# Hitenze/Preconditioned_Additive_Gaussian_Processes_with_Fourier_Acceleration

Measured on AMD Instinct MI355X. Metric: kernel matvecs/sec + PCG wall-time to 1e-6, n=1e6 d=32 additive, 1/2/4/8 GPU, higher is better.
Workload: dtype f64; 1 GPU; additive NFFT matvec, n=1000000, d=32, 32 x 1-D windows, Gaussian f=1 l=1 mu=0.01 (BASELINE configs[2]); n=1000000, d=32, nwindows=32, parallelism=single

## Files before the change

### preconditioned_additive_gaussian_processes_with_fourier_acceleration_amd/csrc/nfft_kernels.hip

```cpp
#include <hip/hip_ext.h>
#include <hip/hip_runtime.h>

#include <algorithm>
#include <cmath>
#include <cstdio>
#include <vector>

#include "internal.h"
#include "reduce.hpp"

namespace nfft4gp_amd {

constexpr int kGridThreads = 1024;
constexpr int kMomStride = kNC + 1;
constexpr int kMomWin = kNC * kNos + 4;
template <int MOMT>
__host__ __device__ constexpr int mom_doubles_per_window()
{
   return MOMT ? kMomWin : kNos * kMomStride;
}
template <int MOMT>
__device__ __forceinline__ int mom_index(int cl, int cell, int d)
{
   return MOMT ? cl * kMomWin + d * kNos + cell : (cl * kNos + cell) * kMomStride + d;
// ... 617 lines not shown
   for (size_t j0 = (size_t)blockIdx.x * kGridThreads + tid; j0 < (size_t)n; j0 += kU * stride) {
      double xv[kU], yv[kU];
#pragma unroll
      for (int u = 0; u < kU; u++) {
         const size_t j = j0 + u * stride;
         xv[u] = j < (size_t)n ? x[j] : 0.0;
         yv[u] = (beta != 0.0 && j < (size_t)n) ? y[j] : 0.0;
      }
#pragma unroll
      for (int u = 0; u < kU; u++) {
         const size_t j = j0 + u * stride;
         if (j < (size_t)n) y[j] = (beta == 0.0 ? 0.0 : beta * yv[u]) + amu * xv[u];
      }
   }
   if (A.bufs) peer_gather(A, comp, s_g);
   __syncthreads();
   grid_tail(comp, s_g, wv, ct, H, s_w, s_h);
}

template <int THREADS, int REC = 5>
__global__ __launch_bounds__(THREADS) void k_interp_part(const uint16_t* __restrict__ meta,
                                                        const uint32_t* __restrict__ lo,
                                                        const uint32_t* __restrict__ qarr,
                                                        const int* __restrict__ tile_off, const double* __restrict__ H,
                                                        double* __restrict__ y, int n, int B, int ngroups, int S,
                                                        double scale)
{
   extern __shared__ __attribute__((aligned(16))) double smem[];
   double* s_y = smem;
   const int b = blockIdx.x / S, part = blockIdx.x % S;
   const int g0 = part * ngroups / S, g1 = (part + 1) * ngroups / S;
   const int tid = threadIdx.x;
   const int base = b * B;
   const int nloc = min(B, n - base);
   TileRegs cur;
   const int t1 = tile_off[b * ngroups + g1];
   int t = tile_at<REC>(cur, meta, lo, qarr, tile_off[b * ngroups + g0] + (tid >> 6), t1);
   for (int i = tid; i < B + kPad; i += THREADS) s_y[i] = 0.0;
   __syncthreads();
   for (; t < t1; t = tile_at<REC>(cur, meta, lo, qarr, t + THREADS / 64, t1)) {
      double h[kNC];
      gather_h(h, H, cur.mt);
      interp_run<REC, false>(cur, h, 0.0);
   }
   __syncthreads();
   for (int j = tid; j < nloc; j += THREADS) atomicAdd(y + (size_t)base + j, scale * s_y[j]);
}

__global__ __launch_bounds__(kGridThreads) void k_reduce_parts(const double* __restrict__ part, int nparts, int nw,
                                                              double* __restrict__ gsum, PeerArgs A)
{
   __shared__ double s_red[kGridThreads];
   const int comp = blockIdx.x;
   const int tid = threadIdx.x;
   const double v = parts_sum(part, nparts, comp, s_red);
   if (tid < kNos) {
      if (A.bufs)
         peer_put(A, comp, tid, v);
      else
         gsum[(size_t)comp * kNos + tid] = v;
   }
}

template <bool GRAD, int THREADS, bool DOT = false, bool DET = false, int REC = 5>
__global__ __launch_bounds__(THREADS) void k_interp(
    const uint16_t* __restrict__ meta, const uint32_t* __restrict__ lo, const uint32_t* __restrict__ qarr,
    const int* __restrict__ tile_off, const double* __restrict__ H, const double* __restrict__ Hd,
    const double* __restrict__ x, double* __restrict__ y, int n, int B, int ngroups, double alpha, double beta,
    double f, double mu, double dg, double* __restrict__ dot_part, unsigned int* __restrict__ dot_ticket,
    double* __restrict__ dot_out, const double* __restrict__ hb, int nw)
{
   extern __shared__ __attribute__((aligned(16))) double smem[];
   const int Bp = B + kPad;
   double* s_y = smem;
   double* s_yd = smem + Bp;
   const int b = blockIdx.x;
   const int tid = threadIdx.x;
   const int base = b * B;
   const int nloc = min(B, n - base);
   if constexpr (GRAD) {
      const int lane = tid & 63;
      const int wave = tid >> 6;
      constexpr int nwaves = THREADS / 64;
      const int t0 = tile_off[b * ngroups];
      const int t1 = tile_off[(b + 1) * ngroups];
      TileRegs cur;
      int t = tile_at<REC>(cur, meta, lo, qarr, t0 + wave, t1);
      const bool ep_regs = B <= kEpMax * THREADS;
      double xe[kEpMax];
      if (ep_regs) {
#pragma unroll
         for (int k = 0; k < kEpMax; k++) {
            const int j = tid + k * THREADS;
            xe[k] = (j < nloc) ? x[(size_t)base + j] : 0.0;
         }
      }
      for (int i = tid; i < Bp; i += THREADS) {
         s_y[i] = 0.0;
         s_yd[i] = 0.0;
      }
      const double Cy = DET ? det_grid(det_interp_exp(hb, nw)) : 0.0;
      const double Cyd = DET ? det_grid(det_interp_exp(hb + nw, nw)) : 0.0;
      __syncthreads();

      for (; t < t1; t += nwaves) {
         const int tn = t + nwaves;
         const size_t hoff = (size_t)cur.mt * kNC;
         double hc[kNC], hdc[kNC];
#pragma unroll
         for (int d = 0; d < kNC; d += 2) {
            const double2 v = *reinterpret_cast<const double2*>(H + hoff + d);
            hc[d] = v.x;
            hc[d + 1] = v.y;
            const double2 vd = *reinterpret_cast<const double2*>(Hd + hoff + d);
            hdc[d] = vd.x;
            hdc[d + 1] = vd.y;
         }
#pragma unroll
         for (int r = 0; r < kR; r++) {
            const uint32_t off = slot_off<REC>(cur, r);
            const double u = q_to_s(cur.qq[r]);
            double v = hc[kNC - 1];
#pragma unroll
            for (int d = kNC - 2; d >= 0; d--) v = fma(v, u, hc[d]);
            lds_add(off, DET ? det_round(v, Cy) : v);
            double vd = hdc[kNC - 1];
#pragma unroll
            for (int d = kNC - 2; d >= 0; d--) vd = fma(vd, u, hdc[d]);
            lds_add(off + 8u * (uint32_t)Bp, DET ? det_round(vd, Cyd) : vd);
         }
         if (tn < t1) load_tile<REC>(cur, meta, lo, qarr, tn, lane);
      }
      __syncthreads();

      const double ff = f * f;
      double* y0 = y;
      double* y1 = y + n;
      double* y2 = y + 2 * (size_t)n;
#pragma unroll
      for (int k = 0; k < kEpMax; k++) {
         if (!ep_regs) break;
         const int j = tid + k * THREADS;
         if (j >= nloc) break;
         const size_t gj = (size_t)base + j;
         const double xj = xe[k];
         const double v0 = 2.0 * f * (s_y[j] + mu * xj);
         const double v1 = ff * s_yd[j];
         const double v2 = dg * ff * xj;
         if (beta == 0.0) {
            y0[gj] = alpha * v0;
            y1[gj] = alpha * v1;
            y2[gj] = alpha * v2;
         } else {
            y0[gj] = fma(beta, y0[gj], alpha * v0);
            y1[gj] = fma(beta, y1[gj], alpha * v1);
            y2[gj] = fma(beta, y2[gj], alpha * v2);
         }
      }
      if (!ep_regs) {
         for (int j = tid; j < nloc; j += THREADS) {
            const size_t gj = (size_t)base + j;
            const double xj = x[gj];
            const double v0 = 2.0 * f * (s_y[j] + mu * xj);
            const double v1 = ff * s_yd[j];
            const double v2 = dg * ff * xj;
            if (beta == 0.0) {
               y0[gj] = alpha * v0;
               y1[gj] = alpha * v1;
               y2[gj] = alpha * v2;
            } else {
               y0[gj] = fma(beta, y0[gj], alpha * v0);
               y1[gj] = fma(beta, y1[gj], alpha * v1);
               y2[gj] = fma(beta, y2[gj], alpha * v2);
            }
         }
      }
      return;
   }
   TileRegs cur;
   const int t1 = tile_off[(b + 1) * ngroups];
   int t = tile_at<REC>(cur, meta, lo, qarr, tile_off[b * ngroups] + (tid >> 6), t1);
   double xe[kEpMax], ye[kEpMax];
   ep_prefetch<THREADS>(xe, ye, x, y, base, nloc, beta);
   for (int i = tid; i < Bp; i += THREADS) s_y[i] = 0.0;
   const double Cy = DET ? det_grid(det_interp_exp(hb, nw)) : 0.0;
   __syncthreads();

   for (; t < t1; t = tile_at<REC>(cur, meta, lo, qarr, t + THREADS / 64, t1)) {
      double h[kNC];
      gather_h(h, H, cur.mt);
      interp_run<REC, DET>(cur, h, Cy);
   }
   __syncthreads();

   const double dacc = ep_plain<THREADS, DOT>(xe, ye, s_y, y, base, nloc, alpha, beta, f, mu);
   if (DOT) ep_dot_finish<THREADS>(dacc, smem + Bp, dot_part, dot_ticket, dot_out);
}

constexpr int kHlWin = kNC * kNos + 1;
constexpr size_t kMaxDynamicLds = 160 * 1024;

__host__ __device__ constexpr size_t hl_lds_bytes(int B, int CG, int ngroups, int ns)
{
   return sizeof(double) * ((size_t)B + kPad) + sizeof(double) * (size_t)ns * CG * kHlWin +
          sizeof(int) * (1 + (size_t)ns + 2 * (size_t)ngroups);
}

__device__ __forceinline__ void hl_stage_wave(double* s_H, const double* __restrict__ H, int g, int slot, int CG, int nw,
                                              int lane)
{
   const int c0 = g * CG;
   const int ncomp = min(CG, nw - c0);
   const double2* src = reinterpret_cast<const double2*>(H + (size_t)c0 * kNos * kNC);
   double* dst = s_H + (size_t)slot * CG * kHlWin;
   const int pairs = ncomp * kNos * kNC / 2;
#pragma unroll 4
   for (int i = lane; i < pairs; i += 64) {
      const double2 v = src[i];
      const int e = 2 * i;
      const int cl = e / (kNos * kNC);
      const int cell = (e / kNC) & (kNos - 1);
      const int d = e & (kNC - 1);
      double* row = dst + cl * kHlWin + cell;
      row[d * kNos] = v.x;
      row[(d + 1) * kNos] = v.y;
   }
}

template <int THREADS, bool DET = false, int REC = 5>
__global__ __launch_bounds__(THREADS) void k_interp_hl(const uint16_t* __restrict__ meta, const uint32_t* __restrict__ lo,
                                                       const uint32_t* __restrict__ qarr, const int* __restrict__ tile_off,
                                                       const double* __restrict__ H, const double* __restrict__ x,
                                                       double* __restrict__ y, int n, int B, int ngroups, int CG, int nw,
                                                       double alpha, double beta, double f, double mu,
                                                       const double* __restrict__ hb, int ns)
{
   extern __shared__ __attribute__((aligned(16))) double smem[];
   const int Bp = B + kPad;
   double* s_y = smem;
   double* s_H = smem + Bp;
   int* s_ready = reinterpret_cast<int*>(s_H + (size_t)ns * CG * kHlWin);
   int* s_done = s_ready + ns;
   int* s_toff = s_done + ngroups;
   const int b = blockIdx.x;
   const int tid = threadIdx.x;
   const int base = b * B;
   const int nloc = min(B, n - base);
   const int lane = tid & 63;
   const int wave = tid >> 6;
   constexpr int nwaves = THREADS / 64;
   const int gbase = b * ngroups;
   TileRegs cur;
   const int t1 = tile_off[gbase + ngroups];
   int t = tile_at<REC>(cur, meta, lo, qarr, tile_off[gbase] + wave, t1);
   double xe[kEpMax], ye[kEpMax];
   ep_prefetch<THREADS>(xe, ye, x, y, base, nloc, beta);
   for (int i = tid; i < Bp; i += THREADS) s_y[i] = 0.0;
   for (int i = tid; i < ngroups; i += THREADS) s_done[i] = 0;
   for (int i = tid; i <= ngroups; i += THREADS) s_toff[i] = tile_off[gbase + i];
   if (tid < ns) s_ready[tid] = tid;
   if (wave < ns && wave < ngroups) hl_stage_wave(s_H, H, wave, wave, CG, nw, lane);
   const double Cy = DET ? det_grid(det_interp_exp(hb, nw)) : 0.0;
   __syncthreads();

   int g = 0, gslot = 0;
   int gend = s_toff[1];
   auto leave = [&](int gl) {
      int old = 0;
      if (lane == 0) old = __hip_atomic_fetch_add(s_done + gl, 1, __ATOMIC_ACQ_REL, __HIP_MEMORY_SCOPE_WORKGROUP);
      old = __builtin_amdgcn_readfirstlane(old);
      if (old == nwaves - 1 && gl + ns < ngroups) {
         const int sl = gl % ns;
         hl_stage_wave(s_H, H, gl + ns, sl, CG, nw, lane);
         __builtin_amdgcn_fence(__ATOMIC_RELEASE, "workgroup");
         if (lane == 0) __hip_atomic_store(s_ready + sl, gl + ns, __ATOMIC_RELEASE, __HIP_MEMORY_SCOPE_WORKGROUP);
      }
   };
   for (; t < t1; t = tile_at<REC>(cur, meta, lo, qarr, t + nwaves, t1)) {
      while (t >= gend) {
         leave(g);
         g++;
         gend = s_toff[g + 1];
         gslot = g % ns;
         if (g >= ns) {
            for (long spin = 0; spin < (1l << 24); spin++) {
               if (__hip_atomic_load(s_ready + gslot, __ATOMIC_ACQUIRE, __HIP_MEMORY_SCOPE_WORKGROUP) == g) break;
               __builtin_amdgcn_s_sleep(1);
            }
         }
      }
      const int cl = (int)(cur.mt >> 6) - g * CG;
      const int cell = (int)(cur.mt & 63u);
      double h[kNC];
      gather_h_lds(h, s_H + ((size_t)gslot * CG + cl) * kHlWin + cell, kNos);
      interp_run<REC, DET>(cur, h, Cy);
   }
   for (; g < ngroups; g++) leave(g);
   __syncthreads();

   ep_plain<THREADS, false>(xe, ye, s_y, y, base, nloc, alpha, beta, f, mu);
}

constexpr int kFgWin = kNC * kFgCells + 1;
constexpr int kFgRow = kNos + 1;
constexpr int kFgQuads = (kFgSpan + 3) / 4;
constexpr int kFgHs = 4 * kFgQuads + 1;
constexpr int kFgLdsWin = kFgWin + kFgHs + 2 * kFgRow;

template <int THREADS, bool DOT = false, int REC = 5, bool TIMELINE = false>
__global__ __launch_bounds__(THREADS) void k_interp_fg(
    const uint16_t* __restrict__ meta, const uint32_t* __restrict__ lo, const uint32_t* __restrict__ qarr,
    const int* __restrict__ tile_off, const double* __restrict__ gsum, double* __restrict__ gclear,
    const double* __restrict__ wcirc, const double* __restrict__ x, double* __restrict__ y, int n, int B, int ngroups,
    double alpha, double beta, double f, double mu, double* __restrict__ dot_part,
    unsigned int* __restrict__ dot_ticket, double* __restrict__ dot_out, int nw)
{
   static_assert(THREADS % (4 * kNC) == 0 && kNC == 8, "a thread keeps its degree and cell quarter over the build");
   static_assert(kFgSpan % 6 == 0, "the circulant's steps go six per trip");
   extern __shared__ __attribute__((aligned(16))) double smem[];
   const int Bp = B + kPad;
   double* s_y = smem;
   double* s_H = smem + Bp;
   double* s_h = s_H + (size_t)nw * kFgWin;
   double* s_g = s_h + (size_t)nw * kFgHs;
   double* s_w = s_g + (size_t)nw * kFgRow;
   double* s_scr = s_w + (size_t)nw * kFgRow;
   const int b = blockIdx.x;
   const int tid = threadIdx.x;
   const int base = b * B;
   const int nloc = min(B, n - base);
   constexpr int nwaves = THREADS / 64;
   if (TIMELINE) stamp(0);
   const int t1 = tile_off[(b + 1) * ngroups];
   int t = tile_off[b * ngroups] + (tid >> 6);
   constexpr int kFgRegTrips = 2;
   const int ns = nw * kNos;
   double gv[kFgRegTrips], wv[kFgRegTrips];
#pragma unroll
   for (int k = 0; k < kFgRegTrips; k++) {
      const int i = min(tid + k * THREADS, ns - 1);
      gv[k] = gsum[i];
      wv[k] = wcirc[i];
   }
   double ct[kTaps];
#pragma unroll
   for (int tp = 0; tp < kTaps; tp++) ct[tp] = c_taps[tp * kNC + (tid & (kNC - 1))];
   for (int i = tid + kFgRegTrips * THREADS; i < ns; i += THREADS) {
      const int o = (i >> 6) * kFgRow + (i & (kNos - 1));
      s_g[o] = gsum[i];
      s_w[o] = wcirc[i];
   }
   TileRegs cur, nxt;
   __builtin_amdgcn_sched_barrier(0);
   load_tile<REC>(cur, meta, lo, qarr, max(min(t, t1 - 1), 0), tid & 63);
   __builtin_amdgcn_sched_barrier(0);
   for (int i = tid; i < Bp; i += THREADS) s_y[i] = 0.0;
#pragma unroll
   for (int k = 0; k < kFgRegTrips; k++) {
      const int i = tid + k * THREADS;
      if (i < ns) {
         const int o = (i >> 6) * kFgRow + (i & (kNos - 1));
         s_g[o] = gv[k];
         s_w[o] = wv[k];
      }
   }
   if (b == 0)
      for (int i = tid; i < ns; i += THREADS) gclear[i] = 0.0;
   __syncthreads();
   if (TIMELINE) stamp(1);
   for (int it = tid; it < nw * kFgQuads; it += THREADS) {
      const int w = it / kFgQuads, k0 = 4 * (it % kFgQuads);
      const double* gw = s_g + w * kFgRow;
      const double* ww = s_w + w * kFgRow;
      double r3 = ww[(k0 + 3) & (kNos - 1)], r2 = ww[(k0 + 2) & (kNos - 1)], r1 = ww[(k0 + 1) & (kNos - 1)], r0 = ww[k0];
      double a0 = 0.0, a1 = 0.0, a2 = 0.0, a3 = 0.0;
#pragma unroll 6
      for (int j = 0; j < kFgSpan; j++) {
         const double gj = gw[(kFgSpan0 + j) & (kNos - 1)];
         a0 = fma(r0, gj, a0);
         a1 = fma(r1, gj, a1);
         a2 = fma(r2, gj, a2);
         a3 = fma(r3, gj, a3);
         r3 = r2, r2 = r1, r1 = r0;
         r0 = ww[(k0 - j - 1) & (kNos - 1)];
      }
      double* hw = s_h + w * kFgHs + k0;
      hw[0] = a0, hw[1] = a1, hw[2] = a2, hw[3] = a3;
   }
   load_tile<REC>(nxt, meta, lo, qarr, max(min(t + nwaves, t1 - 1), 0), tid & 63);
   __syncthreads();
   {
      const int d = tid & (kNC - 1), seg = (tid >> 3) & 3;
      const int c0 = seg ? 8 * seg + 1 : 0, c1 = 8 * seg + 9;
      for (int w = tid >> 5; w < nw; w += THREADS / 32) {
         const double* hw = s_h + w * kFgHs + c0;
         double hv[kTaps + 8];
#pragma unroll
         for (int j = 0; j < kTaps + 8; j++) hv[j] = hw[j];
         double acc[9];
#pragma unroll
         for (int k = 0; k < 9; k++) acc[k] = 0.0;
#pragma unroll
         for (int tp = 0; tp < kTaps; tp++) {
#pragma unroll
            for (int k = 0; k < 9; k++) acc[k] = fma(hv[k + tp], ct[tp], acc[k]);
         }
         double* dst = s_H + (size_t)w * kFgWin + d * kFgCells + c0;
#pragma unroll
         for (int k = 0; k < 9; k++)
            if (c0 + k < c1) dst[k] = acc[k];
      }
   }
   __syncthreads();
   if (TIMELINE) stamp(2);
   double xe[kEpMax], ye[kEpMax];
   ep_prefetch<THREADS>(xe, ye, x, y, base, nloc, beta);

   auto run = [&](const TileRegs& T) {
      const int ci = min((int)((T.mt + 16u) & 63u), kFgCells - 1);
      double h[kNC];
      gather_h_lds(h, s_H + (size_t)(T.mt >> 6) * kFgWin + ci, kFgCells);
      interp_run<REC, false>(T, h, 0.0);
   };
   if (t < t1) {
      run(cur);
      const int tn = t + nwaves;
      t = t1;
      if (tn < t1) {
         t = tile_at<REC>(cur, meta, lo, qarr, tn + nwaves, t1);
         run(nxt);
      }
   }
   for (; t < t1; t = tile_at<REC>(cur, meta, lo, qarr, t + nwaves, t1)) run(cur);
   __syncthreads();
   if (TIMELINE) stamp(3);

   const double dacc = ep_plain<THREADS, DOT, true>(xe, ye, s_y, y, base, nloc, alpha, beta, f, mu);
   if (DOT) ep_dot_finish<THREADS>(dacc, s_scr, dot_part, dot_ticket, dot_out);
}


template <int THREADS, bool DET = false, int REC = 5>
__global__ __launch_bounds__(THREADS) void k_interp2(const uint16_t* __restrict__ meta,
                                                     const uint32_t* __restrict__ lo,
                                                     const uint32_t* __restrict__ qarr,
                                                     const int* __restrict__ tile_off, const double* __restrict__ H,
                                                     size_t h_rs, const double* __restrict__ x0,
                                                     const double* __restrict__ x1, double* __restrict__ y0,
                                                     double* __restrict__ y1, int n, int B, int ngroups, double alpha,
                                                     double beta, double f, double mu, const double* __restrict__ hb,
                                                     int nw)
{
   extern __shared__ __attribute__((aligned(16))) double smem[];
   const int Bp = B + kPad;
   double* s_y0 = smem;
   double* s_y1 = smem + Bp;
   const int b = blockIdx.x;
   const int tid = threadIdx.x;
   const int base = b * B;
   const int nloc = min(B, n - base);
   const int lane = tid & 63;
   const int wave = tid >> 6;
   constexpr int nwaves = THREADS / 64;
   const int t0 = tile_off[b * ngroups];
   const int t1 = tile_off[(b + 1) * ngroups];
   TileRegs cur;
   int t = tile_at<REC>(cur, meta, lo, qarr, t0 + wave, t1);
   for (int i = tid; i < Bp; i += THREADS) s_y0[i] = s_y1[i] = 0.0;
   double C0 = 0.0, C1 = 0.0;
   if (DET) {
      C0 = det_grid(det_interp_exp(hb, nw));
      C1 = det_grid(det_interp_exp(hb + 2 * nw, nw));
   }
   __syncthreads();
   const double* H1 = H + h_rs;
   for (; t < t1; t += nwaves) {
      const size_t hoff = (size_t)cur.mt * kNC;
      double h0[kNC], h1[kNC];
#pragma unroll
      for (int d = 0; d < kNC; d += 2) {
         const double2 v0 = *reinterpret_cast<const double2*>(H + hoff + d);
         const double2 v1 = *reinterpret_cast<const double2*>(H1 + hoff + d);
         h0[d] = v0.x;
         h0[d + 1] = v0.y;
         h1[d] = v1.x;
         h1[d + 1] = v1.y;
      }
#pragma unroll
      for (int r = 0; r < kR; r++) {
         const uint32_t off = slot_off<REC>(cur, r);
         const double u = q_to_s(cur.qq[r]);
         double v0 = h0[kNC - 1], v1 = h1[kNC - 1];
#pragma unroll
         for (int d = kNC - 2; d >= 0; d--) {
            v0 = fma(v0, u, h0[d]);
            v1 = fma(v1, u, h1[d]);
         }
         lds_add(off, DET ? det_round(v0, C0) : v0);
         lds_add(off + 8u * (uint32_t)Bp, DET ? det_round(v1, C1) : v1);
      }
      if (t + nwaves < t1) load_tile<REC>(cur, meta, lo, qarr, t + nwaves, lane);
   }
   __syncthreads();
   const double ff = f * f;
   for (int j = tid; j < nloc; j += THREADS) {
      const size_t gj = (size_t)base + j;
      const double v0 = ff * (s_y0[j] + mu * x0[gj]);
      const double v1 = ff * (s_y1[j] + mu * x1[gj]);
      y0[gj] = (beta == 0.0) ? alpha * v0 : fma(beta, y0[gj], alpha * v0);
      y1[gj] = (beta == 0.0) ? alpha * v1 : fma(beta, y1[gj], alpha * v1);
   }
}

template <typename F, typename... A>
static void launch_ev(F fn, dim3 grid, dim3 block, size_t lds, hipStream_t s, const hipEvent_t* ev, A... args)
{
   if (ev)
      hipExtLaunchKernelGGL(fn, grid, block, (std::uint32_t)lds, s, ev[0], ev[1], 0u, args...);
   else
      hipLaunchKernelGGL(fn, grid, block, lds, s, args...);
}

static int spread_momt(const AdditivePlan& P) { return P.spread_variant == 2 ? 0 : 1; }

static size_t spread_lds_bytes(const AdditivePlan& P)
{
   const size_t per = spread_momt(P) ? mom_doubles_per_window<1>() : mom_doubles_per_window<0>();
   return sizeof(double) * ((size_t)P.B + kPad + (size_t)P.CG * per) + (P.det ? 64 : 0);
}

constexpr size_t kRedScratch = sizeof(double) * (2 * (1024 / 64) + 1);

static size_t interp_lds_bytes(const AdditivePlan& P, int grad)
{
   return sizeof(double) * ((size_t)P.B + kPad) * (grad ? 2 : 1) + kRedScratch;
}

int upload_tap_coeffs()
{
   static bool done[64] = {false};
   int dev = 0;
   NFFT4GP_HIP_CHECK(hipGetDevice(&dev));
   if (dev < 0 || dev >= 64) return -1;
   if (!done[dev]) {
      NFFT4GP_HIP_CHECK(hipMemcpyToSymbol(HIP_SYMBOL(c_taps_u), tap_poly_coeffs().data(), sizeof(double) * kTaps * kNC));
      std::vector<double> C = tap_poly_coeffs();
      for (int t = 0; t < kTaps; t++)
         for (int d = 0; d < kNC; d++) C[t * kNC + d] = std::ldexp(C[t * kNC + d], -32 * d);
      NFFT4GP_HIP_CHECK(hipMemcpyToSymbol(HIP_SYMBOL(c_taps), C.data(), sizeof(double) * kTaps * kNC));
      done[dev] = true;
   }
   return 0;
}

typedef void (*SpreadFn)(const uint16_t*, const uint32_t*, const uint32_t*, const int*, const int*, const double*, int,
                         int, int, int, int, int, double*, double*, int);
constexpr int kSpreadThreads = 512;
static const SpreadFn kSpreadFns[2][2][4] = {
    {{k_spread<kSpreadThreads>, k_spread<kSpreadThreads, true>, k_spread<kSpreadThreads, false, 0>,
      k_spread<kSpreadThreads, false, 1, false, 5, true>},
     {k_spread<kSpreadThreads, false, 1, true>, k_spread<kSpreadThreads, true, 1, true>,
      k_spread<kSpreadThreads, false, 0, true>, k_spread<kSpreadThreads, false, 1, true, 5, true>}},
    {{k_spread<kSpreadThreads, false, 1, false, 4>, k_spread<kSpreadThreads, true, 1, false, 4>,
      k_spread<kSpreadThreads, false, 0, false, 4>, k_spread<kSpreadThreads, false, 1, false, 4, true>},
     {k_spread<kSpreadThreads, false, 1, true, 4>, k_spread<kSpreadThreads, true, 1, true, 4>,
      k_spread<kSpreadThreads, false, 0, true, 4>, k_spread<kSpreadThreads, false, 1, true, 4, true>}}};
constexpr int kNumSpreadVariants = 4;
constexpr size_t kInfinityCacheBytes = 256ull << 20;
int pick_spread_variant(const AdditivePlan& P)
{
   int v = P.spread_variant;
   if (v < 0) v = P.dl.bytes > kInfinityCacheBytes ? 3 : 0;
   return std::min(v, kNumSpreadVariants - 1);
}
static SpreadFn spread_fn(const AdditivePlan& P)
{
   return kSpreadFns[P.rec == 4 ? 1 : 0][P.det ? 1 : 0][pick_spread_variant(P)];
}

constexpr int kInterpThreads = 1024;
typedef void (*InterpFn)(const uint16_t*, const uint32_t*, const uint32_t*, const int*, const double*,
                         const double*, const double*, double*, int, int, int, double, double, double, double,
                         double, double*, unsigned int*, double*, const double*, int);

template <int T, int REC>
static InterpFn interp_fn_t(bool grad, bool dot, bool det)
{
   if (grad) return det ? k_interp<true, T, false, true, REC> : k_interp<true, T, false, false, REC>;
   if (dot) return det ? k_interp<false, T, true, true, REC> : k_interp<false, T, true, false, REC>;
   return det ? k_interp<false, T, false, true, REC> : k_interp<false, T, false, false, REC>;
}
static InterpFn interp_fn(bool grad, bool dot, bool small, bool det, int rec)
{
   if (rec == 4) return small ? interp_fn_t<512, 4>(grad, dot, det) : interp_fn_t<kInterpThreads, 4>(grad, dot, det);
   return small ? interp_fn_t<512, 5>(grad, dot, det) : interp_fn_t<kInterpThreads, 5>(grad, dot, det);
}
constexpr int kInterp2Threads = 1024;
typedef void (*Interp2Fn)(const uint16_t*, const uint32_t*, const uint32_t*, const int*, const double*, size_t,
                          const double*, const double*, double*, double*, int, int, int, double, double, double, double,
                          const double*, int);
template <int REC>
static Interp2Fn interp2_fn_t(bool det, bool small)
{
   if (small) return det ? k_interp2<512, true, REC> : k_interp2<512, false, REC>;
   return det ? k_interp2<kInterp2Threads, true, REC> : k_interp2<kInterp2Threads, false, REC>;
}
static Interp2Fn interp2_fn(bool det, bool small, int rec)
{
   return rec == 4 ? interp2_fn_t<4>(det, small) : interp2_fn_t<5>(det, small);
}
typedef void (*InterpPartFn)(const uint16_t*, const uint32_t*, const uint32_t*, const int*, const double*, double*, int,
                             int, int, int, double);
static InterpPartFn interp_part_fn(int rec) { return rec == 4 ? k_interp_part<512, 4> : k_interp_part<512, 5>; }

typedef void (*InterpFgFn)(const uint16_t*, const uint32_t*, const uint32_t*, const int*, const double*, double*,
                           const double*, const double*, double*, int, int, int, double, double, double, double,
                           double*, unsigned int*, double*, int);
static InterpFgFn interp_fg_fn(bool dot, int rec, bool tl)
{
   if (tl && !dot)
      return rec == 4 ? k_interp_fg<kInterpThreads, false, 4, true> : k_interp_fg<kInterpThreads, false, 5, true>;
   if (rec == 4) return dot ? k_interp_fg<kInterpThreads, true, 4> : k_interp_fg<kInterpThreads, false, 4>;
   return dot ? k_interp_fg<kInterpThreads, true, 5> : k_interp_fg<kInterpThreads, false, 5>;
}

typedef void (*InterpHlFn)(const uint16_t*, const uint32_t*, const uint32_t*, const int*, const double*, const double*,
                           double*, int, int, int, int, int, double, double, double, double, const double*, int);
static InterpHlFn interp_hl_fn(bool small, bool det, int rec)
{
   if (rec == 4)
      return small ? (det ? k_interp_hl<512, true, 4> : k_interp_hl<512, false, 4>)
                   : (det ? k_interp_hl<1024, true, 4> : k_interp_hl<1024, false, 4>);
   return small ? (det ? k_interp_hl<512, true, 5> : k_interp_hl<512, false, 5>)
                : (det ? k_interp_hl<1024, true, 5> : k_interp_hl<1024, false, 5>);
}
bool pick_interp_hl(const AdditivePlan& P)
{
   static const int v = getenv("NFFT4GP_AMD_INTERP_HL") ? atoi(getenv("NFFT4GP_AMD_INTERP_HL")) : -1;
   return (v < 0 ? P.dl.bytes > kInfinityCacheBytes : v != 0) && P.ngroups >= 1;
}
int pick_interp_threads(const AdditivePlan& P)
{
   static const int forced = getenv("NFFT4GP_AMD_INTERP_THREADS") ? atoi(getenv("NFFT4GP_AMD_INTERP_THREADS")) : 0;
   return forced == 512 || (forced != 1024 && P.nblocks >= 512) ? 512 : kInterpThreads;
}
int pick_hl_slots(const AdditivePlan& P)
{
   static const int slots_env = getenv("NFFT4GP_AMD_HL_SLOTS") ? atoi(getenv("NFFT4GP_AMD_HL_SLOTS")) : 0;
   int ns = std::max(2, std::min(slots_env > 0 ? slots_env : 2, pick_interp_threads(P) == 512 ? 2 : 6));
   while (ns > 2 && hl_lds_bytes(P.B, P.CG, P.ngroups, ns) > kMaxDynamicLds) ns--;
   return ns;
}
int pick_interp2_threads()
{
   static const int forced = getenv("NFFT4GP_AMD_INTERP2_THREADS") ? atoi(getenv("NFFT4GP_AMD_INTERP2_THREADS")) : 0;
   return forced == 512 ? 512 : kInterp2Threads;
}

static std::vector<const void*> interp_kernels()
{
   std::vector<const void*> v;
   for (int sm = 0; sm < 2; sm++)
      for (int det = 0; det < 2; det++)
         for (int rec = 4; rec <= 5; rec++) v.push_back((const void*)interp_hl_fn(sm, det, rec));
   for (int g = 0; g < 2; g++)
      for (int d = 0; d < 2; d++)
         for (int sm = 0; sm < 2; sm++)
            for (int det = 0; det < 2; det++)
               for (int rec = 4; rec <= 5; rec++) v.push_back((const void*)interp_fn(g, d && !g, sm, det, rec));
   for (int det = 0; det < 2; det++)
      for (int sm = 0; sm < 2; sm++)
         for (int rec = 4; rec <= 5; rec++) v.push_back((const void*)interp2_fn(det, sm, rec));
   for (int rec = 4; rec <= 5; rec++) v.push_back((const void*)interp_part_fn(rec));
   for (int d = 0; d < 2; d++)
      for (int rec = 4; rec <= 5; rec++)
         for (int tl = 0; tl < 2; tl++) v.push_back((const void*)interp_fg_fn(d, rec, tl));
   return v;
}
static std::vector<const void*> spread_kernels()
{
   std::vector<const void*> v;
   for (const auto& byrec : kSpreadFns)
      for (const auto& bydet : byrec)
         for (const SpreadFn f : bydet) v.push_back((const void*)f);
   return v;
}

static bool lds_ready()
{
   static const bool ok = [] {
      std::vector<const void*> v = interp_kernels();
      for (const void* f : spread_kernels()) v.push_back(f);
      for (const void* f : v)
         (void)hipFuncSetAttribute(f, hipFuncAttributeMaxDynamicSharedMemorySize, (int)kMaxDynamicLds);
      (void)hipGetLastError();
      hipFuncAttributes a;
      for (const void* f : v)
         if (hipFuncGetAttributes(&a, f) != hipSuccess || a.sharedSizeBytes != 0) return false;
      return true;
   }();
   if (!ok) fprintf(stderr, "nfft4gp_amd: a matvec kernel has static LDS; its absolute LDS addressing would be wrong\n");
   return ok;
}

static int launch_spread_to(const AdditivePlan& P, const double* d_x, double* d_part, double* d_gsum,
                            hipStream_t stream)
{
   if (P.dl.ntiles == 0 || P.n == 0) return 0;
   if (!lds_ready()) return -1;
   const SpreadFn fn = spread_fn(P);
   const int gridx = ((P.nblocks + 7) / 8) * 8 * P.ngroups;
   launch_ev(fn, dim3(gridx), dim3(kSpreadThreads), spread_lds_bytes(P), stream, P.kev ? P.kev + 0 : nullptr,
             P.dl.meta, P.dl.lo, P.dl.q, P.dl.tile_off, (const int*)P.dl.cmax, d_x, P.n, P.B, P.nblocks, P.ngroups,
             P.CG, P.nw, d_part, d_gsum, P.spread_fold);
// ... 204 lines not shown
```

Before: 15640 matvecs/s.

## Build fine-grid windows per wave with wave-local sync instead of block barriers

```diff
diff --git a/preconditioned_additive_gaussian_processes_with_fourier_acceleration_amd/csrc/nfft_kernels.hip b/preconditioned_additive_gaussian_processes_with_fourier_acceleration_amd/csrc/nfft_kernels.hip
--- a/preconditioned_additive_gaussian_processes_with_fourier_acceleration_amd/csrc/nfft_kernels.hip
+++ b/preconditioned_additive_gaussian_processes_with_fourier_acceleration_amd/csrc/nfft_kernels.hip
@@ -943,10 +943,108 @@
 }
 
 constexpr int kFgWin = kNC * kFgCells + 1;
-constexpr int kFgRow = kNos + 1;
-constexpr int kFgQuads = (kFgSpan + 3) / 4;
-constexpr int kFgHs = 4 * kFgQuads + 1;
-constexpr int kFgLdsWin = kFgWin + kFgHs + 2 * kFgRow;
+constexpr int kFgG = 3;
+constexpr int kFgGroups = kFgSpan / kFgG;
+constexpr int kFgHalf = 22;
+constexpr int kFgAuxG = 2 * kFgHalf;
+constexpr int kFgAuxW = 4 * kFgHalf;
+constexpr int kFgWoff = 2 * kFgHalf - 1;
+constexpr int kFgWx = kFgSpan + kFgWoff;
+constexpr int kFgAux = 175;
+constexpr int kFgLdsWin = kFgWin + kFgAux;
+static_assert(kFgSpan == kFgG * kFgGroups && 2 * kFgGroups <= 32 && 2 * kFgHalf >= kFgSpan, "the circulant's lanes");
+static_assert(kFgAuxW + kFgWx <= kFgAux && kFgCells + kTaps <= kFgAuxG + 1, "a window's rows fit");
+static_assert(kFgWx <= 2 * kNos, "wx: every entry written by one of a lane's two stores");
+
+__device__ __forceinline__ void wave_lds_sync()
+{
+   __builtin_amdgcn_fence(__ATOMIC_RELEASE, "wavefront");
+   __builtin_amdgcn_wave_barrier();
+   __builtin_amdgcn_fence(__ATOMIC_ACQUIRE, "wavefront");
+}
+__device__ __forceinline__ double lds_ld(const double* p) { return *(const volatile lds_f64*)p; }
+__device__ __forceinline__ double lane_xor1(double v)
+{
+   const int lo = __builtin_amdgcn_mov_dpp(__double2loint(v), 0xB1, 0xF, 0xF, true);
+   const int hi = __builtin_amdgcn_mov_dpp(__double2hiint(v), 0xB1, 0xF, 0xF, true);
+   return __hiloint2double(hi, lo);
+}
+
+__device__ __forceinline__ void fg_stage_window(double* aux, int lane, double g, double w)
+{
+   const int j = (lane - kFgSpan0) & (kNos - 1);
+   if (j < 2 * kFgHalf) aux[kFgAuxG + j] = j < kFgSpan ? g : 0.0;
+   const int m = (lane + kFgWoff) & (kNos - 1);
+   aux[kFgAuxW + m] = w;
+   if (m + kNos < kFgWx) aux[kFgAuxW + m + kNos] = w;
+}
+
+__device__ __forceinline__ void fg_circulant_pair(double* s_a, int w0, int nw, int lane)
+{
+   const int p = lane >> 5, hf = lane & 1, q = min((lane & 31) >> 1, kFgGroups - 1);
+   const bool ok = w0 + 16 * p < nw && (lane & 31) < 2 * kFgGroups;
+   double* aux = s_a + (size_t)(w0 + 16 * p < nw ? w0 + 16 * p : w0) * kFgAux;
+   const double* gw = aux + kFgAuxG + kFgHalf * hf;
+   const double* ww = aux + kFgAuxW + kFgWoff + kFgG * q - kFgHalf * hf;
+   double r[kFgG], a[kFgG];
+#pragma unroll
+   for (int i = 0; i < kFgG; i++) r[i] = lds_ld(ww + i), a[i] = 0.0;
+   constexpr int kBatch = kFgHalf / 2;
+#pragma unroll
+   for (int s0 = 0; s0 < kFgHalf; s0 += kBatch) {
+      double gj[kBatch], wn[kBatch];
+#pragma unroll
+      for (int s = 0; s < kBatch; s++) {
+         gj[s] = lds_ld(gw + s0 + s);
+         wn[s] = s0 + s + 1 < kFgHalf ? lds_ld(ww - (s0 + s) - 1) : 0.0;
+      }
+#pragma unroll
+      for (int s = 0; s < kBatch; s++) {
+#pragma unroll
+         for (int i = 0; i < kFgG; i++) a[i] = fma(r[i], gj[s], a[i]);
+#pragma unroll
+         for (int i = kFgG - 1; i > 0; i--) r[i] = r[i - 1];
+         r[0] = wn[s];
+      }
+   }
+   double h[kFgG];
+#pragma unroll
+   for (int i = 0; i < kFgG; i++) {
+      const double o = lane_xor1(a[i]);
+      h[i] = hf ? o + a[i] : a[i] + o;
+   }
+   static_assert(kFgG == 3, "the stores below");
+   if (ok) {
+      double* hw = aux + kFgG * q;
+      if (hf == 0) hw[0] = h[0];
+      hw[1 + hf] = hf ? h[2] : h[1];
+   }
+}
+
+__device__ __forceinline__ void fg_hbuild_pair(const double* s_a, double* s_H, const double (&ct)[kTaps], int w0,
+                                               int nw, int lane)
+{
+   const int w = w0 + 16 * (lane >> 5);
+   if (w >= nw) return;
+   const int d = lane & (kNC - 1), seg = (lane >> 3) & 3;
+   const int c0 = seg ? 8 * seg + 1 : 0;
+   const double* hw = s_a + (size_t)w * kFgAux + c0;
+   double hv[kTaps + 8];
+#pragma unroll
+   for (int j = 0; j < kTaps + 8; j++) hv[j] = lds_ld(hw + j);
+   double acc[9];
+#pragma unroll
+   for (int k = 0; k < 9; k++) acc[k] = 0.0;
+#pragma unroll
+   for (int tp = 0; tp < kTaps; tp++) {
+#pragma unroll
+      for (int k = 0; k < 9; k++) acc[k] = fma(hv[k + tp], ct[tp], acc[k]);
+   }
+   double* dst = s_H + (size_t)w * kFgWin + d * kFgCells + c0;
+#pragma unroll
+   for (int k = 0; k < 8; k++) dst[k] = acc[k];
+   if (seg == 0) dst[8] = acc[8];
+}
 
 template <int THREADS, bool DOT = false, int REC = 5, bool TIMELINE = false>
 __global__ __launch_bounds__(THREADS) void k_interp_fg(
@@ -956,18 +1054,17 @@
     double alpha, double beta, double f, double mu, double* __restrict__ dot_part,
     unsigned int* __restrict__ dot_ticket, double* __restrict__ dot_out, int nw)
 {
-   static_assert(THREADS % (4 * kNC) == 0 && kNC == 8, "a thread keeps its degree and cell quarter over the build");
-   static_assert(kFgSpan % 6 == 0, "the circulant's steps go six per trip");
+   static_assert(THREADS == 16 * 64 && kNC == 8, "sixteen waves share out the windows; a lane keeps its degree");
    extern __shared__ __attribute__((aligned(16))) double smem[];
    const int Bp = B + kPad;
    double* s_y = smem;
    double* s_H = smem + Bp;
-   double* s_h = s_H + (size_t)nw * kFgWin;
-   double* s_g = s_h + (size_t)nw * kFgHs;
-   double* s_w = s_g + (size_t)nw * kFgRow;
-   double* s_scr = s_w + (size_t)nw * kFgRow;
+   double* s_a = s_H + (size_t)nw * kFgWin;
+   double* s_scr = s_a + (size_t)nw * kFgAux;
    const int b = blockIdx.x;
    const int tid = threadIdx.x;
+   const int lane = tid & 63;
+   const int wave = __builtin_amdgcn_readfirstlane(tid >> 6);
    const int base = b * B;
    const int nloc = min(B, n - base);
    constexpr int nwaves = THREADS / 64;
@@ -975,82 +1072,43 @@
    const int t1 = tile_off[(b + 1) * ngroups];
    int t = tile_off[b * ngroups] + (tid >> 6);
    constexpr int kFgRegTrips = 2;
-   const int ns = nw * kNos;
    double gv[kFgRegTrips], wv[kFgRegTrips];
 #pragma unroll
    for (int k = 0; k < kFgRegTrips; k++) {
-      const int i = min(tid + k * THREADS, ns - 1);
+      const int i = min(wave + k * nwaves, nw - 1) * kNos + lane;
       gv[k] = gsum[i];
       wv[k] = wcirc[i];
    }
    double ct[kTaps];
 #pragma unroll
    for (int tp = 0; tp < kTaps; tp++) ct[tp] = c_taps[tp * kNC + (tid & (kNC - 1))];
-   for (int i = tid + kFgRegTrips * THREADS; i < ns; i += THREADS) {
-      const int o = (i >> 6) * kFgRow + (i & (kNos - 1));
-      s_g[o] = gsum[i];
-      s_w[o] = wcirc[i];
-   }
    TileRegs cur, nxt;
    __builtin_amdgcn_sched_barrier(0);
-   load_tile<REC>(cur, meta, lo, qarr, max(min(t, t1 - 1), 0), tid & 63);
+   load_tile<REC>(cur, meta, lo, qarr, max(min(t, t1 - 1), 0), lane);
    __builtin_amdgcn_sched_barrier(0);
    for (int i = tid; i < Bp; i += THREADS) s_y[i] = 0.0;
 #pragma unroll
    for (int k = 0; k < kFgRegTrips; k++) {
-      const int i = tid + k * THREADS;
-      if (i < ns) {
-         const int o = (i >> 6) * kFgRow + (i & (kNos - 1));
-         s_g[o] = gv[k];
-         s_w[o] = wv[k];
-      }
+      const int w = wave + k * nwaves;
+      if (w < nw) fg_stage_window(s_a + (size_t)w * kFgAux, lane, gv[k], wv[k]);
    }
    if (b == 0)
-      for (int i = tid; i < ns; i += THREADS) gclear[i] = 0.0;
-   __syncthreads();
+      for (int i = tid; i < nw * kNos; i += THREADS) gclear[i] = 0.0;
+   wave_lds_sync();
    if (TIMELINE) stamp(1);
-   for (int it = tid; it < nw * kFgQuads; it += THREADS) {
-      const int w = it / kFgQuads, k0 = 4 * (it % kFgQuads);
-      const double* gw = s_g + w * kFgRow;
-      const double* ww = s_w + w * kFgRow;
-      double r3 = ww[(k0 + 3) & (kNos - 1)], r2 = ww[(k0 + 2) & (kNos - 1)], r1 = ww[(k0 + 1) & (kNos - 1)], r0 = ww[k0];
-      double a0 = 0.0, a1 = 0.0, a2 = 0.0, a3 = 0.0;
-#pragma unroll 6
-      for (int j = 0; j < kFgSpan; j++) {
-         const double gj = gw[(kFgSpan0 + j) & (kNos - 1)];
-         a0 = fma(r0, gj, a0);
-         a1 = fma(r1, gj, a1);
-         a2 = fma(r2, gj, a2);
-         a3 = fma(r3, gj, a3);
-         r3 = r2, r2 = r1, r1 = r0;
-         r0 = ww[(k0 - j - 1) & (kNos - 1)];
-      }
-      double* hw = s_h + w * kFgHs + k0;
-      hw[0] = a0, hw[1] = a1, hw[2] = a2, hw[3] = a3;
-   }
-   load_tile<REC>(nxt, meta, lo, qarr, max(min(t + nwaves, t1 - 1), 0), tid & 63);
-   __syncthreads();
-   {
-      const int d = tid & (kNC - 1), seg = (tid >> 3) & 3;
-      const int c0 = seg ? 8 * seg + 1 : 0, c1 = 8 * seg + 9;
-      for (int w = tid >> 5; w < nw; w += THREADS / 32) {
-         const double* hw = s_h + w * kFgHs + c0;
-         double hv[kTaps + 8];
-#pragma unroll
-         for (int j = 0; j < kTaps + 8; j++) hv[j] = hw[j];
-         double acc[9];
-#pragma unroll
-         for (int k = 0; k < 9; k++) acc[k] = 0.0;
-#pragma unroll
-         for (int tp = 0; tp < kTaps; tp++) {
-#pragma unroll
-            for (int k = 0; k < 9; k++) acc[k] = fma(hv[k + tp], ct[tp], acc[k]);
-         }
-         double* dst = s_H + (size_t)w * kFgWin + d * kFgCells + c0;
-#pragma unroll
-         for (int k = 0; k < 9; k++)
-            if (c0 + k < c1) dst[k] = acc[k];
-      }
+   if (wave < nw) fg_circulant_pair(s_a, wave, nw, lane);
+   load_tile<REC>(nxt, meta, lo, qarr, max(min(t + nwaves, t1 - 1), 0), lane);
+   if (wave < nw) {
+      wave_lds_sync();
+      fg_hbuild_pair(s_a, s_H, ct, wave, nw, lane);
+   }
+   const int w3 = wave + kFgRegTrips * nwaves;
+   if (w3 < nw) {
+      fg_stage_window(s_a + (size_t)w3 * kFgAux, lane, gsum[w3 * kNos + lane], wcirc[w3 * kNos + lane]);
+      wave_lds_sync();
+      fg_circulant_pair(s_a, w3, nw, lane);
+      wave_lds_sync();
+      fg_hbuild_pair(s_a, s_H, ct, w3, nw, lane);
    }
    __syncthreads();
    if (TIMELINE) stamp(2);
```

Result: no change. 15790 matvecs/s, median of 6 (+1.0%).
